# orybkin/video-gcp

Measured on AMD Instinct MI355X. Metric: predicted frames/sec, 64x64x3 seq_len=80 gcp_tree (posterior forward + all loss terms, model(inputs) and model.loss() of train.py:157-159, batch-stat BatchNorm), higher is better.
Workload: dtype f32 (encoder / decoder convs and the tree GEMMs from 512 rows: split-f16 MFMA with f32 accumulate, f32-equivalent; everything else exact f32 MFMA)

## Files before the change

### video-gcp_amd/csrc/conv3x3_split.hip

```cpp
#include "common.h"
#include "split_mfma.h"

#include <cstdlib>
#include <type_traits>

namespace {

struct SplitUpCfg {
    static constexpr int RW = 18, RH = 6, LW = 10, LH = 4, CC = 16, KS = 5;
    static constexpr int RAW_BYTES = LH * LW * CC * 4;
    static constexpr int PLANE_BYTES = RH * RW * 32;
    static constexpr int WAVE_BYTES = RAW_BYTES + 2 * PLANE_BYTES;
    static constexpr int NS = (LH * LW * 4 + 63) / 64;
    static constexpr int W_CHUNK_BYTES = KS * 2 * 1024;
    static int lds_bytes(int nchunk) { return nchunk * W_CHUNK_BYTES + 8 * WAVE_BYTES + 8 * 2 * 16 * 4; }
};

__global__ void __launch_bounds__(512, 2) conv3x3_up16_split_kernel(const gcpx_conv_args a, const int items_per_wave,
                                                                    const int nitems) {
    using Cfg = SplitUpCfg;
    constexpr int RW = Cfg::RW, RH = Cfg::RH, LW = Cfg::LW, LH = Cfg::LH, CC = Cfg::CC, NS = Cfg::NS, KS = Cfg::KS;
    extern __shared__ float4 smem4[];
    const int nchunk = a.Cin / CC;
    const char* wl = reinterpret_cast<const char*>(smem4);
// ... 163 lines not shown
            const int which = tid >> 4, c = tid & 15;
            float sum = 0.f;
#pragma unroll
            for (int w = 0; w < 8; ++w) sum += red[(w * 2 + which) * 16 + c];
            a.stats_partial[((size_t)blockIdx.x * 2 + which) * 16 + c] = sum;
        }
    }
}

template <int TILE> struct SplitTileShape;
template <> struct SplitTileShape<1> { static constexpr int TH = 16, TW = 16, TF = 1; };
template <> struct SplitTileShape<2> { static constexpr int TH = 8, TW = 8, TF = 4; };

template <int CT, int TILE>
struct SplitTileCfg {
    using TS = SplitTileShape<TILE>;
    static constexpr int TH = TS::TH, TW = TS::TW, TF = TS::TF, CC = 32, C4 = 8;
    static constexpr int RH = TH + 2, RW = TW + 2, LH = TH / 2 + 2, LW = TW / 2 + 2;
    static constexpr int PLANE_BYTES = TF * RH * RW * 64;
    static constexpr int RAW_BYTES = TF * LH * LW * CC * 4;
    static constexpr int LDS_BYTES = 2 * PLANE_BYTES + RAW_BYTES + 64;
    static constexpr int NSLOT = TF * LH * LW * C4;
    static constexpr int NS = (NSLOT + 255) / 256;
    static constexpr int PR = TH * TW * TF / 64;
};

template <int CT, int TILE>
__global__ void __launch_bounds__(256, 2) conv3x3_up32_split_kernel(const gcpx_conv_args a, const int ntx, const int nty, const int ntiles) {
    using Cfg = SplitTileCfg<CT, TILE>;
    constexpr int PR = Cfg::PR, TH = Cfg::TH, TW = Cfg::TW, TF = Cfg::TF, RH = Cfg::RH, RW = Cfg::RW;
    constexpr int LH = Cfg::LH, LW = Cfg::LW, CC = Cfg::CC, C4 = Cfg::C4, NS = Cfg::NS, NSLOT = Cfg::NSLOT;
    static_assert(PR == 4, "256 output pixels per workgroup");
    extern __shared__ float4 smem4[];
    char* hi = reinterpret_cast<char*>(smem4);
    float* raw = reinterpret_cast<float*>(hi + 2 * Cfg::PLANE_BYTES);
    float* wmax = reinterpret_cast<float*>(hi + 2 * Cfg::PLANE_BYTES + Cfg::RAW_BYTES);

    const int tid = threadIdx.x;
    const int lane = tid & 63, wave = tid >> 6;
    const int j = lane & 15, q = lane >> 4;
    const int nchunk = a.Cin / CC;
    const int Hout = a.Hout, Wout = a.Wout, F = a.F;
    const int ew = a.w_split_log2_dev ? __builtin_amdgcn_readfirstlane(*a.w_split_log2_dev) : a.w_split_log2;

    int pixoff[PR], pfl[PR], py[PR], px[PR];
#pragma unroll
    for (int pt = 0; pt < PR; ++pt) {
        const int p = (wave * PR + pt) * 16 + j;
        pfl[pt] = p / (TH * TW);
        const int rem = p % (TH * TW);
        py[pt] = rem / TW;
        px[pt] = rem % TW;
        pixoff[pt] = ((pfl[pt] * RH + py[pt]) * RW + px[pt]) * 64 + q * 16;
    }
    auto slot = [&](int k, int& c4, int& rx, int& ry, int& fl, int& lds) {
        const int idx = tid + 256 * k;
        c4 = idx % C4;
        int t = idx / C4;
        rx = t % LW; t /= LW;
        ry = t % LH;
        fl = (idx < NSLOT) ? t / LH : -1;
        lds = ((fl * LH + ry) * LW + rx) * CC + c4 * 4;
    };
    const char* wbase = reinterpret_cast<const char*>(a.wpk_split) + lane * 16;
    const int nstep = nchunk * 9;

    f32x4 st1[CT], st2[CT];
#pragma unroll
    for (int ct = 0; ct < CT; ++ct) { st1[ct] = f32x4{0, 0, 0, 0}; st2[ct] = f32x4{0, 0, 0, 0}; }

    float4 pre[NS];
    unsigned pre_ok = 0;
    auto tile_origin = [&](int tile, int& f0, int& y0, int& x0) {
        const int tx = tile % ntx;
        const int t2 = tile / ntx;
        f0 = (t2 / nty) * TF; y0 = (t2 % nty) * TH; x0 = tx * TW;
    };
    auto issue_loads = [&](int tile, int chunk) {
        int f0, y0, x0;
        tile_origin(tile, f0, y0, x0);
        pre_ok = 0;
        const int c0 = a.src[0].C;
#pragma unroll
        for (int k = 0; k < NS; ++k) {
            pre[k] = make_float4(0.f, 0.f, 0.f, 0.f);
            int s_c4, s_rx, s_ry, s_fl, s_lds;
            slot(k, s_c4, s_rx, s_ry, s_fl, s_lds);
            if (s_fl < 0) continue;
            const int f = f0 + s_fl;
            if (f < F) {
                const int sy = min(max(y0 / 2 - 1 + s_ry, 0), a.Hin - 1);
                const int sx = min(max(x0 / 2 - 1 + s_rx, 0), a.Win - 1);
                const int cg = chunk * CC + s_c4 * 4;
                const bool first = cg < c0;
                const gcpx_conv_src& sr = first ? a.src[0] : a.src[1];
                const int cl = first ? cg : cg - c0;
                pre[k] = *reinterpret_cast<const float4*>(sr.ptr + (((size_t)(f / sr.frame_div) * a.Hin + sy) * a.Win + sx) * sr.C + cl);
                pre_ok |= 1u << k;
            }
        }
    };

    int tile = blockIdx.x;
    if (tile < ntiles) issue_loads(tile, 0);
    for (; tile < ntiles; tile += gridDim.x) {
        int f0, y0, x0;
        tile_origin(tile, f0, y0, x0);
        f32x4 acc[CT][PR];
#pragma unroll
        for (int ct = 0; ct < CT; ++ct)
#pragma unroll
            for (int pt = 0; pt < PR; ++pt) acc[ct][pt] = f32x4{0, 0, 0, 0};
        int ex = 0;
        const bool top = (y0 == 0), bot = (y0 + TH == Hout), lft = (x0 == 0), rgt = (x0 + TW == Wout);

        h8 wr[3][CT][2];
        auto wload = [&](const int stn_, h8 (&w)[CT][2]) __attribute__((always_inline)) {
            const char* wp = wbase + (size_t)min(stn_, nstep - 1) * CT * 2048;
#pragma unroll
            for (int ct = 0; ct < CT; ++ct) {
                w[ct][0] = *reinterpret_cast<const h8*>(wp + ct * 2048);
                w[ct][1] = *reinterpret_cast<const h8*>(wp + ct * 2048 + 1024);
            }
        };
        if constexpr (CT <= 2) {
            wload(0, wr[0]);
            wload(1, wr[1]);
        }

        for (int chunk = 0; chunk < nchunk; ++chunk) {
            float amax = 0.f;
            {
                const int c0 = a.src[0].C;
#pragma unroll
                for (int k = 0; k < NS; ++k) {
                    int s_c4, s_rx, s_ry, s_fl, s_lds;
                    slot(k, s_c4, s_rx, s_ry, s_fl, s_lds);
                    if (s_fl < 0) continue;
                    float4 v = pre[k];
                    if (pre_ok & (1u << k)) {
                        const int cg = chunk * CC + s_c4 * 4;
                        const bool first = cg < c0;
                        const gcpx_conv_src& sr = first ? a.src[0] : a.src[1];
                        v = affine_act4(v, sr.scale, sr.shift, first ? cg : cg - c0, sr.act);
                    }
                    *reinterpret_cast<float4*>(raw + s_lds) = v;
                    amax = fmaxf(amax, fmaxf(fmaxf(fabsf(v.x), fabsf(v.y)), fmaxf(fabsf(v.z), fabsf(v.w))));
                }
            }
#pragma unroll
            for (int m = 1; m < 64; m <<= 1) amax = fmaxf(amax, __shfl_xor(amax, m));
            if (lane == 0) wmax[wave] = amax;
            __syncthreads();
            amax = fmaxf(fmaxf(wmax[0], wmax[1]), fmaxf(wmax[2], wmax[3]));
            int ec = 14 + 127 - (int)((__float_as_uint(amax) >> 23) & 0xff);
            ec = __builtin_amdgcn_readfirstlane(amax > 0.f ? max(-100, min(min(100, 126 - ew), ec)) : min(100, 126 - ew));
            if (chunk == 0) ex = ec;
            else if (ec < ex) {
                const float r = __uint_as_float((unsigned)(127 + ec - ex) << 23);
#pragma unroll
                for (int ct = 0; ct < CT; ++ct)
#pragma unroll
                    for (int pt = 0; pt < PR; ++pt) acc[ct][pt] *= r;
                ex = ec;
            }
            const float sx2 = __uint_as_float((unsigned)(127 + ex) << 23);
            {
                const int c4 = tid & (C4 - 1);
                const int p = tid >> 3;
                constexpr int RPP = 32 / (TW * TF);
                const int fl = (TF > 1) ? p / TW : 0;
                const int rx = p % TW;
                const int rsub = (RPP == 2) ? (p / TW) : 0;
                auto lerp_store = [&](int f2, int ry, int cx, bool zero) {
                    const float wx1 = (cx & 1) ? 0.75f : 0.25f, wx0 = 1.f - wx1;
                    const float wy1 = ((ry & 1) ? 0.75f : 0.25f), wy0 = 1.f - wy1;
                    const float* r = raw + ((f2 * LH + (ry >> 1)) * LW + (cx >> 1)) * CC + c4 * 4;
                    const float4 a00 = *reinterpret_cast<const float4*>(r);
                    const float4 a01 = *reinterpret_cast<const float4*>(r + CC);
                    const float4 a10 = *reinterpret_cast<const float4*>(r + LW * CC);
                    const float4 a11 = *reinterpret_cast<const float4*>(r + LW * CC + CC);
                    float4 v;
                    v.x = wy0 * (wx0 * a00.x + wx1 * a01.x) + wy1 * (wx0 * a10.x + wx1 * a11.x);
                    v.y = wy0 * (wx0 * a00.y + wx1 * a01.y) + wy1 * (wx0 * a10.y + wx1 * a11.y);
// ... 5 lines not shown
                    p1[0] = (_Float16)v.x; p1[1] = (_Float16)v.y; p1[2] = (_Float16)v.z; p1[3] = (_Float16)v.w;
                    p2[0] = (_Float16)(v.x - (float)p1[0]); p2[1] = (_Float16)(v.y - (float)p1[1]);
                    p2[2] = (_Float16)(v.z - (float)p1[2]); p2[3] = (_Float16)(v.w - (float)p1[3]);
                    char* dst = hi + ((f2 * RH + ry) * RW + cx) * 64 + c4 * 8;
                    *reinterpret_cast<h4*>(dst) = p1;
                    *reinterpret_cast<h4*>(dst + Cfg::PLANE_BYTES) = p2;
                };
#pragma unroll 2
                for (int k = 0; k < RH / RPP; ++k) {
                    const int ry = k * RPP + rsub;
                    lerp_store(fl, ry, rx + 1, (top && ry == 0) || (bot && ry == RH - 1));
                }
                for (int e = p; e < TF * RH * 2; e += 32) {
                    const int side = e & 1;
                    const int ry = (e >> 1) % RH, f2 = (e >> 1) / RH;
                    lerp_store(f2, ry, side ? RW - 1 : 0,
                               (top && ry == 0) || (bot && ry == RH - 1) || (lft && side == 0) || (rgt && side == 1));
                }
            }
            __syncthreads();
            if (chunk + 1 < nchunk) issue_loads(tile, chunk + 1);
            else if (tile + (int)gridDim.x < ntiles) issue_loads(tile + gridDim.x, 0);

            if constexpr (CT <= 2) {
                auto tap_mfmas = [&](const int tap, const h8 (&wc)[CT][2]) __attribute__((always_inline)) {
                    const int tapoff = ((tap / 3) * RW + (tap % 3)) * 64;
                    h8 b1[PR], b2[PR];
    #pragma unroll
                    for (int pt = 0; pt < PR; ++pt) {
                        b1[pt] = *reinterpret_cast<const h8*>(hi + pixoff[pt] + tapoff);
                        b2[pt] = *reinterpret_cast<const h8*>(hi + pixoff[pt] + tapoff + Cfg::PLANE_BYTES);
                    }
    #pragma unroll
                    for (int ct = 0; ct < CT; ++ct) {
    #pragma unroll
                        for (int pt = 0; pt < PR; ++pt) acc[ct][pt] = mfma32h(wc[ct][1], b1[pt], acc[ct][pt]);
    #pragma unroll
                        for (int pt = 0; pt < PR; ++pt) acc[ct][pt] = mfma32h(wc[ct][0], b2[pt], acc[ct][pt]);
    #pragma unroll
                        for (int pt = 0; pt < PR; ++pt) acc[ct][pt] = mfma32h(wc[ct][0], b1[pt], acc[ct][pt]);
                    }
                };
                __builtin_amdgcn_s_setprio(1);
    #pragma unroll 1
                for (int t3 = 0; t3 < 9; t3 += 3) {
                    wload(chunk * 9 + t3 + 2, wr[2]);
                    tap_mfmas(t3, wr[0]);
                    wload(chunk * 9 + t3 + 3, wr[0]);
                    tap_mfmas(t3 + 1, wr[1]);
                    wload(chunk * 9 + t3 + 4, wr[1]);
                    tap_mfmas(t3 + 2, wr[2]);
                }
            } else {
                h8 wn[CT][2];
                {
                    const char* wp = wbase + (size_t)(chunk * 9) * CT * 2048;
    #pragma unroll
                    for (int ct = 0; ct < CT; ++ct) {
                        wn[ct][0] = *reinterpret_cast<const h8*>(wp + ct * 2048);
                        wn[ct][1] = *reinterpret_cast<const h8*>(wp + ct * 2048 + 1024);
                    }
                }
                __builtin_amdgcn_s_setprio(1);
    #pragma unroll 1
                for (int tap = 0; tap < 9; ++tap) {
                    const int tapoff = ((tap / 3) * RW + (tap % 3)) * 64;
                    h8 wc[CT][2];
    #pragma unroll
                    for (int ct = 0; ct < CT; ++ct) { wc[ct][0] = wn[ct][0]; wc[ct][1] = wn[ct][1]; }
                    {
                        const int stn = min(chunk * 9 + tap + 1, nstep - 1);
                        const char* wp = wbase + (size_t)stn * CT * 2048;
    #pragma unroll
                        for (int ct = 0; ct < CT; ++ct) {
                            wn[ct][0] = *reinterpret_cast<const h8*>(wp + ct * 2048);
                            wn[ct][1] = *reinterpret_cast<const h8*>(wp + ct * 2048 + 1024);
                        }
                    }
                    h8 b1[PR], b2[PR];
    #pragma unroll
                    for (int pt = 0; pt < PR; ++pt) {
                        b1[pt] = *reinterpret_cast<const h8*>(hi + pixoff[pt] + tapoff);
                        b2[pt] = *reinterpret_cast<const h8*>(hi + pixoff[pt] + tapoff + Cfg::PLANE_BYTES);
                    }
    #pragma unroll
                    for (int ct = 0; ct < CT; ++ct) {
    #pragma unroll
                        for (int pt = 0; pt < PR; ++pt) acc[ct][pt] = mfma32h(wc[ct][1], b1[pt], acc[ct][pt]);
    #pragma unroll
                        for (int pt = 0; pt < PR; ++pt) acc[ct][pt] = mfma32h(wc[ct][0], b2[pt], acc[ct][pt]);
    #pragma unroll
                        for (int pt = 0; pt < PR; ++pt) acc[ct][pt] = mfma32h(wc[ct][0], b1[pt], acc[ct][pt]);
                    }
                }
            }
            __builtin_amdgcn_s_setprio(0);
        }

        const float inv = __uint_as_float((unsigned)(127 - ex - ew) << 23);
#pragma unroll
        for (int pt = 0; pt < PR; ++pt) {
            const int f = f0 + pfl[pt];
            if (f >= F) continue;
            float* op = a.out + (((size_t)f * Hout + (y0 + py[pt])) * Wout + (x0 + px[pt])) * a.out_pitch;
#pragma unroll
            for (int ct = 0; ct < CT; ++ct) {
                const float4 bv = *reinterpret_cast<const float4*>(a.bias + ct * 16 + q * 4);
                f32x4 v = acc[ct][pt];
                v[0] = fmaf(v[0], inv, bv.x); v[1] = fmaf(v[1], inv, bv.y); v[2] = fmaf(v[2], inv, bv.z); v[3] = fmaf(v[3], inv, bv.w);
                if (a.addend) {
                    const float4 ad = *reinterpret_cast<const float4*>(a.addend + (((size_t)(f / a.addend_frame_div) * Hout + (y0 + py[pt])) * Wout +
                                                                                   (x0 + px[pt])) * a.out_pitch + ct * 16 + q * 4);
                    v[0] += ad.x; v[1] += ad.y; v[2] += ad.z; v[3] += ad.w;
                }
                *reinterpret_cast<float4*>(op + ct * 16 + q * 4) = make_float4(v[0], v[1], v[2], v[3]);
                if (a.stats_partial) {
                    st1[ct] += v;
                    st2[ct] += v * v;
                }
            }
        }
    }

    if (a.stats_partial) {
        __syncthreads();
        float* red = reinterpret_cast<float*>(hi);
#pragma unroll
        for (int ct = 0; ct < CT; ++ct) {
#pragma unroll
            for (int r = 0; r < 4; ++r) {
                const float s1 = row16_sum(st1[ct][r]);
                const float s2 = row16_sum(st2[ct][r]);
                if (j == 0) {
                    red[(wave * 2 + 0) * CT * 16 + ct * 16 + q * 4 + r] = s1;
                    red[(wave * 2 + 1) * CT * 16 + ct * 16 + q * 4 + r] = s2;
                }
            }
        }
        __syncthreads();
        if (tid < 2 * CT * 16) {
            const int which = tid / (CT * 16), c = tid % (CT * 16);
            float sum = 0.f;
#pragma unroll
            for (int w = 0; w < 4; ++w) sum += red[(w * 2 + which) * CT * 16 + c];
            a.stats_partial[((size_t)blockIdx.x * 2 + which) * CT * 16 + c] = sum;
        }
    }
}

template <int CT, int TILE>
int launch_up32_split(const gcpx_conv_args* a, hipStream_t stream, int grid) {
    using Cfg = SplitTileCfg<CT, TILE>;
    const int ntx = a->Wout / Cfg::TW, nty = a->Hout / Cfg::TH;
    const int nfg = (a->F + Cfg::TF - 1) / Cfg::TF;
    auto kern = conv3x3_up32_split_kernel<CT, TILE>;
    static bool attr_set = false;
    if (!attr_set) {
        hipError_t e = hipFuncSetAttribute(reinterpret_cast<const void*>(kern), hipFuncAttributeMaxDynamicSharedMemorySize, Cfg::LDS_BYTES);
        if (e != hipSuccess) {
            gcpx_set_error("conv3x3 split up32: hipFuncSetAttribute(%d B LDS): %s", Cfg::LDS_BYTES, hipGetErrorString(e));
            return GCPX_ERR_HIP;
        }
        attr_set = true;
    }
    hipLaunchKernelGGL(kern, dim3(grid), dim3(256), Cfg::LDS_BYTES, stream, *a, ntx, nty, ntx * nty * nfg);
    GCPX_CHECK_LAUNCH();
    return GCPX_OK;
// ... 946 lines not shown
```

### video-gcp_amd/forward_plan.py

```python
import ctypes as C
import os
from contextlib import contextmanager

import torch

from . import packing as pk
from . import runtime as rt
from .hparams import GCPHParams
from .params import init_params, encoder_layers, encoder_skip_layers, decoder_layers
from .plan_ops import _Plan, _addr, N_LANES


class ForwardPlanMixin:

    def _plan_encoder(self, plan, tag, x_ptr, F, out_ptr, out_ob, out_orow, out_rpb):
        hp, P, lib = self._hp, self.pk, self.lib
        G = lib.gcpx_conv4x4s2_grid()
        S = hp.img_sz
        skip_idx = encoder_skip_layers(hp)
        skips = {}
        a0 = self._buf(f"{tag}.a0", (F, S // 2, S // 2, hp.ngf))
        enc_rec = dict(F=F, x_ptr=x_ptr, a0=a0, r={}, out=(out_ptr, out_ob, out_orow, out_rpb))
        plan.rec[f"enc:{tag}"] = enc_rec
        plan.add(f"enc.input:{tag}", lib.gcpx_conv4x4s2_image, x_ptr, P["enc.input.w"].data_ptr(),
# ... 47 lines not shown
        T, nz, dk = hp.max_seq_len, hp.nz_enc, hp.nz_attn_key
        li = l if hp.untied_layers else 0
        qin = self._buf(f"attn.qin{l}", (M, dk))
        self._mlp(plan, f"attn.query{l}", W["attn.query"], [el, er], M, n, out=qin.data_ptr(), ob=n * dk, orow=dk)
        dense = lambda t, w: self._rowsrc(t.data_ptr(), 0, w, w)
        qp = self._buf(f"attn.q{l}", (M, dk))
        self._gemm(plan, f"attn.q_proj{l}", [dense(qin, dk)], M, dk, M, W["attn.q_proj.w"], W["attn.q_proj.b"],
                   out=qp.data_ptr(), ob=0, orow=dk)
        o = self._buf(f"attn.o{l}", (M, nz))
        gamma = self._buf(f"attn.gamma{l}", (M, T))
        temp = self.sd[f"tree_module.tree_modules.{li}.inference.attention.attention_layers.0.temperature"]
        plan.add(f"attn{l}", lib.gcpx_attention, qp.data_ptr(), _addr(Kp, li * B * T * dk), _addr(Vp, li * B * T * nz), None,
                 tin["end_ind"].data_ptr(), temp.data_ptr(), o.data_ptr(), gamma.data_ptr(), M, n, T, dk, nz, hp.n_attention_heads)
        raw = self._buf(f"attn.raw{l}", (M, nz))
        self._gemm(plan, f"attn.out_proj{l}", [dense(o, nz)], M, nz, M, W["attn.out_proj.w"], W["attn.out_proj.b"],
                   out=raw.data_ptr(), ob=0, orow=nz)
        et = self._buf(f"attn.e_tilde{l}", (M, nz))
        self._gemm(plan, f"attn.out{l}", [dense(raw, nz)], M, nz, M, W["attn.out.w"], W["attn.out.b"], out=et.data_ptr(), ob=0, orow=nz)
        plan.rec.setdefault("gamma", {})[l] = gamma
        plan.rec.setdefault("e_tilde", {})[l] = et
        plan.rec.setdefault("attn", {})[l] = dict(qin=qin, qp=qp, o=o, raw=raw, gamma=gamma, et=et, M=M, n=n, li=li, temp=temp)
        return self._rowsrc(et.data_ptr(), n * nz, nz, nz)

    def _plan_decoder_features(self, plan, e_src, F, rpb, skips):
        hp, P, lib = self._hp, self.pk, self.lib
        ctop = self._c_top
        d0 = self._buf("dec.d0", (F, 4, 4, ctop))
        plan.rec["dec"] = dict(F=F, rpb=rpb, e_src=e_src, d0=d0, blocks=[], skips=skips)
        nrb = lib.gcpx_gemm_row_blocks(F, 16 * ctop)
        st = self._buf("dec.st0", (nrb, 2, 16 * ctop)) if self.training else None
        self._gemm(plan, "dec.input", [e_src], F, 16 * ctop, rpb, P["dec.input.w"], P["dec.input.b"], out=d0.data_ptr(),
                   ob=rpb * 16 * ctop, orow=16 * ctop, stats=st)
        sc, sh = self._bn(plan, "dec.bn0", "decoder.net.input.norm", ctop, st, nrb, 16 * ctop, F * 16)
        prev = (d0.data_ptr(), ctop, 1, sc, sh, rt.ACT_LRELU)
        res = 4
        for name, c_prev, c_skip, skip_idx, cout in decoder_layers(hp):
            srcs = [prev]
            if skip_idx >= 0:
                t, C_, ssc, ssh, sact = skips[skip_idx]
                assert C_ == c_skip and t.shape[1] == res
                srcs.append((t.data_ptr(), C_, rpb, ssc, ssh, sact))
            o = self._buf(f"dec.{name}", (F, 2 * res, 2 * res, cout))
            cpad = (cout + 15) // 16 * 16
            hoist = (skip_idx >= 0 and rpb > 1 and F % rpb == 0 and self.split_f16 and cout in (32, 64) and c_prev % 32 == 0 and
                     c_skip % 32 == 0 and f"dec.{name}" in self.pk_split and "fold" not in self.pk_split[f"dec.{name}"] and
                     os.environ.get("GCPX_NO_SKIP_HOIST") is None)
            hoist16 = (skip_idx >= 0 and rpb > 1 and F % rpb == 0 and self.split_f16 and cout == 16 and c_prev == 16 and c_skip == 16 and
                       f"dec.{name}.f16a" in self.pk_split and res % 4 == 0 and os.environ.get("GCPX_NO_SKIP_HOIST") is None)
            addend = None
            if hoist or hoist16:
                addend = self._buf(f"dec.{name}.skip", (F // rpb, 2 * res, 2 * res, cout))
                t, C_, ssc, ssh, sact = skips[skip_idx]
                zb = self._buf(f"dec.{name}.zero_bias", (cpad,), zero=True)
                a_s = self._conv_args([(t.data_ptr(), C_, 1, ssc, ssh, sact)], F // rpb, res, res, 2 * res, 2 * res, cout, cout,
                                      P[f"dec.{name}.w"], zb, addend, upsample=1)
                if hoist16:
                    self._set_split(a_s, f"dec.{name}.f16b")
                else:
                    self._set_split(a_s, f"dec.{name}")
                    a_s.wpk_split = a_s.wpk_split + (c_prev // 32) * 9 * (cpad // 16) * 2048
                plan.keep.append(a_s)
                plan.add(f"dec.{name}.skip", lib.gcpx_conv3x3, C.byref(a_s))
                srcs_main = [prev]
            else:
                srcs_main = srcs
            a = self._conv_args(srcs_main, F, res, res, 2 * res, 2 * res, cout, cout, P[f"dec.{name}.w"], P[f"dec.{name}.b"],
                                o, upsample=1, stats=(o if self.training else None))
            if hoist or hoist16:
                a.addend, a.addend_frame_div = addend.data_ptr(), rpb
            self._set_split(a, f"dec.{name}.f16a" if hoist16 else f"dec.{name}")
            Gl = lib.gcpx_conv3x3_grid(C.byref(a))
            assert Gl > 0, rt.lib().gcpx_last_error()
            st = self._buf(f"dec.st.{name}", (Gl, 2, cpad)) if self.training else None
            a.stats_partial = st.data_ptr() if st is not None else None
            plan.keep.append(a)
            plan.add(f"dec.{name}", lib.gcpx_conv3x3, C.byref(a))
            plan.rec["dec"]["blocks"].append(dict(name=name, srcs=srcs, out=o, res_in=res, cout=cout, c_prev=c_prev, c_skip=c_skip,
                                                  skip_idx=skip_idx))
            res *= 2
            sc, sh = self._bn(plan, f"dec.bn.{name}", f"decoder.net.{name}.norm", cout, st, Gl, cpad, F * res * res)
            prev = (o.data_ptr(), cout, 1, sc, sh, rt.ACT_LRELU)
        assert res == hp.img_sz
        return prev

    def _build_plan(self, key, tin):
        hp, P, lib = self._hp, self.pk, self.lib
        B, has_traj, has_z, sample_prior, phase, pred_len = key.B, key.has_traj, key.has_z, key.sample_prior, key.phase, key.pred_len
        train_aux = has_traj and phase == "train" and not sample_prior
        L, T, N = hp.hierarchy_levels, hp.max_seq_len, hp.n_nodes
        nz, nv, H, SD = hp.nz_enc, hp.nz_vae, hp.nz_mid_lstm, hp.lstm_state_dim
        PS = 2 ** L + 1
        plan = _Plan(lib)
        G = lib.gcpx_conv_grid()
# ... 55 lines not shown
                    else:
                        kenc = self._buf("inf_key_enc", (B * T, nz))
                        self._plan_seq_encoder(plan, "kseq", "inf_key_encoder.0", enc_traj, kenc, B)
                    keys = self._buf("inf_enc_key_seq", (B * T, dk))
                    dense = lambda t, w: self._rowsrc(t.data_ptr(), 0, w, w)
                    self._gemm(plan, "kseq.key", [dense(kenc, nz)], B * T, dk, B * T, P["kseq.key.w"], P["kseq.key.b"],
                               out=keys.data_ptr(), ob=0, orow=dk)
                    Kp = self._buf("attn.K", (n_mod, B * T, dk))
                    Vp = self._buf("attn.V", (n_mod, B * T, nz))
                    self._gemm(plan, "attn.k_proj", [dense(keys, dk)], B * T, dk, B * T, P["attn.k_proj.w"], P["attn.k_proj.b"],
                               out=Kp.data_ptr(), ob=0, orow=dk, batch=(n_mod, 0, P["attn.k_proj.w"][0].numel(), dk, B * T * dk))
                    self._gemm(plan, "attn.v_proj", [dense(inf_enc, nz)], B * T, nz, B * T, P["attn.v_proj.w"], P["attn.v_proj.b"],
                               out=Vp.data_ptr(), ob=0, orow=nz, batch=(n_mod, 0, P["attn.v_proj.w"][0].numel(), nz, B * T * nz))
                    plan.rec["attn_kv"] = dict(Kp=Kp, Vp=Vp, keys=keys, kenc=kenc, n_mod=n_mod)

        if traj_first:
            plan_traj_encoder()
        plan.lane = 1
        if "rng_all" in tin:
            plan.add("randn", lib.gcpx_randn, tin["rng_all"].data_ptr(), tin["rng_all"].numel(), self._buf("rng_state", (2,), torch.int64).data_ptr())
            if "aux_n" in tin and not pred_len:
                plan.wait(2, 1)
        skips = self._plan_encoder(plan, "I0", tin["I_0"].data_ptr(), B, _addr(E), PS * nz, 0, 1)
        plan.lane = 2
        if not pred_len:
            if "aux_n" in tin:
                plan_aux_indices()
            plan_bookkeeping()
        if hp.attach_cost_mdl and hp.run_cost_mdl and train_aux and self._has_aux_training:
            gt = self._buf("cost_target", (B,))
            rows = hp.input_nc * hp.img_sz
            plan.add("path_cost", lib.gcpx_path_cost, tin["traj_seq"].data_ptr(), tin["cost_start_idx"].data_ptr(),
                     tin["cost_end_idx"].data_ptr(), B, T, rows, hp.img_sz, self._buf("cost_partial", (B, rows)).data_ptr(), gt.data_ptr())
        self._plan_encoder(plan, "Ig", tin["I_g"].data_ptr(), B, _addr(E, 2 ** L * nz), PS * nz, 0, 1)
        outs = {}
        e0 = lambda: self._rowsrc(_addr(E), PS * nz, 0, nz)
        eg = lambda: self._rowsrc(_addr(E, 2 ** L * nz), PS * nz, 0, nz)
        if hp.regress_length and not pred_len:
            plan.wait(2, 1)
            logits = self._buf("seq_len_logits", (B, T))
            self._mlp(plan, "length_pred", P["length_pred"], [e0(), eg()], B, 1, out=logits.data_ptr(), ob=T, orow=0)
            outs["seq_len_logits"] = logits
        if not traj_first:
            plan_traj_encoder()
        plan.lane = 0
        plan.join([1, 2])
# ... 191 lines not shown
            la.seq_len = seq_len.data_ptr()
            if "actions_sampled" in outs and "actions" in tin:
                la.action_pred, la.action_seq, la.inv_t0 = outs["actions_sampled"].data_ptr(), tin["actions"].data_ptr(), tin["inv_t0"].data_ptr()
                la.n_actions, la.w_action = hp.n_actions, hp.action_rec_weight
            if "cost_pred" in outs:
                la.cost_pred, la.cost_target, la.w_cost = outs["cost_pred"].data_ptr(), outs["cost_target"].data_ptr(), 1.0
            loss_out = self._buf("losses", (16,), zero=True)
            la.out, la.B, la.T, la.N, la.state_dim = loss_out.data_ptr(), B, T, (N - 1 if adaptive else N), hp.state_dim
            la.w_rec, la.w_kl, la.w_len, la.w_exist, la.w_state = hp.dense_img_rec_weight, hp.kl_weight, hp.length_pred_weight, 1.0, 1.0
            if self._kl_w is not None:
                la.w_kl_dev = self._kl_w.data_ptr()
            la.total_div = float(T * hp.input_nc * hp.img_sz * hp.img_sz)
            plan.keep.append(la)
            return la, kl_b

        decode, with_loss = key.decode, key.with_loss
        loss_pre = None
        if with_loss and not adaptive:
            loss_pre = loss_args()
            plan.add("loss.pre", lib.gcpx_loss_pre, C.byref(loss_pre[0]), *kl_args(loss_pre[1]))
        if decode:
            F = B * N
            S = hp.img_sz
            prev = self._plan_decoder_features(plan, self._rowsrc(_addr(E, nz), PS * nz, nz, nz), F, N, skips)
            images = self._buf("images_df", (B, N, hp.input_nc, S, S))
            distr = matched_distr = None
            dlm = hp.decoder_distribution == "discrete_logistic_mixture"
            head_out, row_map = None, None
            fused_nll = None
            if dlm:
                mode = rt.HEAD_DLM_MEAN
                if self.materialize_distr or (adaptive and self.save_for_backward and with_loss):
                    mode, distr = rt.HEAD_DLM_BOTH, self._buf("distr_df", (B, N, S, S, self._head_pitch))
                    head_out = distr
                elif self._head_grad_fused(key):
                    mode, row_map = rt.HEAD_DLM_NLL_GRAD, node2row
                    head_out = self._buf("bw.dMD", (B * T, S, S, self._head_pitch))
                    fused_nll = self._buf("nll_partial", ((S // 4) * (S // 16), B * T), zero=True)
                    plan.rec["nll_bwd_fused"] = plan.rec["head_grad_fused"] = True
                elif with_loss and not adaptive and not self.save_for_backward and self._head_nll_fusable():
                    mode, row_map = rt.HEAD_DLM_NLL, node2row
                    fused_nll = self._buf("nll_partial", ((S // 4) * (S // 16), B * T), zero=True)
                elif with_loss and not adaptive:
                    mode, matched_distr = rt.HEAD_DLM_BOTH, self._buf("matched_distr", (B, T, S, S, self._head_pitch))
                    head_out, row_map = matched_distr, node2row
            else:
                mode = rt.HEAD_TANH_NCHW
# ... 122 lines not shown
```

### video-gcp_amd/sequential.py

```python
import ctypes as C
import os

import torch

from . import runtime as rt
from .model import GCPTreeModel, Outputs, _Plan, _addr
from .params import init_params_sequential


class GCPSequentialModel(GCPTreeModel):
    _has_aux_training = True
    _has_pred_length = False
    _rng_in_plan = False
    _has_training = True

    def _check_hp(self, hp):
        assert hp.lstm_init in ("zero", "mlp")
        assert hp.n_actions <= 16 or not hp.action_conditioned_pred, "the action rows are padded to one 16-column k-group"

    @property
    def _nets(self):
        return ("gen_lstm",) if self._hp.deterministic else ("prior_lstm", "inf_lstm", "gen_lstm")

    def _default_params(self, hp, seed):
# ... 131 lines not shown
        hp, P, lib = self._hp, self.pk, self.lib
        B, has_traj, has_z, sample_prior, phase, with_loss = key.B, key.has_traj, key.has_z, key.sample_prior, key.phase, key.with_loss
        T, nz, nv, H, nl = hp.max_seq_len, hp.nz_enc, hp.nz_vae, hp.nz_mid_lstm, hp.n_lstm_layers
        S = hp.img_sz
        plan = _Plan(lib)
        X = self._buf("seq.X", (B, T, nz))
        EG = self._buf("seq.EG", (B, nz))
        PZ = self._buf("seq.PZ", (B, T - 1, 2 * nv))
        QZ = self._buf("seq.QZ", (B, T - 1, 2 * nv), zero=True)
        Z = self._buf("seq.Z", (B, T - 1, nv))
        idx = self._buf("seq.idx", (B, T), torch.int32)
        seq_len = self._buf("seq.len", (B,), torch.int32)
        plan.add("seq_index", lib.gcpx_seq_index, tin["end_ind"].data_ptr(), B, T, idx.data_ptr(), seq_len.data_ptr())
        train_aux = has_traj and phase == "train" and not sample_prior
        if "aux_n" in tin:
            AUXK = ("inv_t0", "inv_t1", "cost_start_idx", "cost_end_idx")
            plan.add("aux_sample_indices", lib.gcpx_aux_sample_indices_gauss, tin["end_ind"].data_ptr(), tin["aux_n"].data_ptr(), B,
                     hp.inv_mdl_temp_dist, *[tin[k].data_ptr() for k in AUXK])

        enc_traj = None
        plan.fork([1, 2])
        plan.lane = 1
        skips = self._plan_encoder(plan, "I0", tin["I_0"].data_ptr(), B, _addr(X), T * nz, 0, 1)
        plan.lane = 2
        if hp.attach_cost_mdl and hp.run_cost_mdl and train_aux and "cost_start_idx" in tin:
            rows = hp.input_nc * hp.img_sz
            plan.add("path_cost", lib.gcpx_path_cost, tin["traj_seq"].data_ptr(), tin["cost_start_idx"].data_ptr(),
                     tin["cost_end_idx"].data_ptr(), B, T, rows, hp.img_sz, self._buf("cost_partial", (B, rows)).data_ptr(),
                     self._buf("cost_target", (B,)).data_ptr())
        self._plan_encoder(plan, "Ig", tin["I_g"].data_ptr(), B, _addr(EG), nz, 0, 1)
        plan.lane = 0
        if has_traj:
            enc_traj = self._buf("enc_traj", (B * T, nz))
            self._plan_encoder(plan, "traj", tin["traj_seq"].data_ptr(), B * T, enc_traj.data_ptr(), T * nz, nz, T)
        plan.join([1, 2])
        outs = {}
        e0 = lambda: self._rowsrc(_addr(X), T * nz, 0, nz)
        eg = lambda: self._rowsrc(_addr(EG), nz, 0, nz)
        if hp.regress_length:
            logits = self._buf("seq_len_logits", (B, T))
            self._mlp(plan, "length_pred", P["length_pred"], [e0(), eg()], B, 1, out=logits.data_ptr(), ob=T, orow=0)
            outs["seq_len_logits"] = logits

        EA = None
        if hp.action_conditioned_pred:
            na = hp.n_actions
# ... 174 lines not shown
            first = enc_traj if has_traj else mes
            s0 = self._rowsrc(first.data_ptr(), T * nz, nz, nz)
            s1 = self._rowsrc(_addr(mes, nz), T * nz, nz, nz)
            self._mlp(plan, "inv_mdl", P["inv_mdl"], [s0, s1], B * (T - 1), T - 1, out=act.data_ptr(),
                      ob=(T - 1) * hp.n_actions, orow=hp.n_actions)
            outs["actions_padded"] = act
        if aux_ok and ((hp.attach_inv_mdl and not hp.train_inv_mdl_full_seq) or (hp.attach_cost_mdl and hp.run_cost_mdl)):
            aux_rows = self._buf("aux_rows", (4, B), torch.int32)
            plan.add("aux_index_rows", lib.gcpx_aux_index_rows, tin["inv_t0"].data_ptr(), tin["inv_t1"].data_ptr(),
                     tin["cost_start_idx"].data_ptr(), tin["cost_end_idx"].data_ptr(), B, T, T, aux_rows.data_ptr())
            gather = lambda t, i: self._rowsrc(t.data_ptr(), 0, nz, nz, rowidx=aux_rows[i])
            if hp.attach_inv_mdl and not hp.train_inv_mdl_full_seq:
                act = self._buf("actions_sampled", (B, hp.n_actions))
                self._mlp(plan, "inv_mdl", P["inv_mdl"], [gather(enc_traj, 0), gather(mes, 1)], B, B, out=act.data_ptr(), ob=0,
                          orow=hp.n_actions)
                outs["actions_sampled"] = act
            if hp.attach_cost_mdl and hp.run_cost_mdl:
                cost = self._buf("cost_pred", (B, 1))
                self._mlp(plan, "cost_mdl", P["cost_mdl"], [gather(mes, 2), gather(mes, 3)], B, B, out=cost.data_ptr(), ob=0, orow=1)
                outs["cost_pred"], outs["cost_target"] = cost, self._buf("cost_target", (B,))
        plan.lane = 0

        F = B * (T - 1)
        prev = self._plan_decoder_features(plan, self._rowsrc(_addr(X, nz), T * nz, nz, nz), F, T - 1, skips)
        dec_images = self._buf("seq.dec_images", (B, T - 1, hp.input_nc, S, S))
        dlm = hp.decoder_distribution == "discrete_logistic_mixture"
        head_out = row_map = matched = fused_nll = None
        if dlm:
            mode = rt.HEAD_DLM_MEAN
            if with_loss or self.materialize_distr:
                row_map = self._buf("seq.row_map", (F,), torch.int32)
                row_map.copy_((torch.arange(B)[:, None] * T + torch.arange(1, T)[None]).reshape(-1).to(torch.int32))
                if with_loss and self._head_nll_fusable():
                    fused_nll = self._buf("nll_partial", ((S // 4) * (S // 16), B * T), zero=True)
                    mode = rt.HEAD_DLM_NLL
                    if self.save_for_backward:
                        mode, head_out = rt.HEAD_DLM_NLL_GRAD, self._buf("bw.dMD", (B * T, S, S, self._head_pitch))
                        r2f = self._buf("seq.row2frame", (B * T,), torch.int32)
                        inv = torch.arange(B * T, dtype=torch.int64).view(B, T) // T * (T - 1) + torch.arange(T)[None] - 1
                        inv[:, 0] = -1
                        r2f.copy_(inv.reshape(-1).to(torch.int32))
                        plan.add("zero_unmapped", lib.gcpx_zero_unmapped_rows, head_out.data_ptr(), S * S * self._head_pitch,
                                 r2f.data_ptr(), B * T)
                        plan.rec["nll_bwd_fused"] = plan.rec["head_grad_fused"] = True
                else:
                    mode, matched = rt.HEAD_DLM_BOTH, self._buf("matched_distr", (B, T, S, S, self._head_pitch))
                    head_out = matched
# ... 123 lines not shown
```

Before: 503,700.

## Split up32 conv output channels across wavefronts and hoist decoder skip convs earlier

The 32-channel upsample conv kernel now splits output-channel tiles across wavefronts when CT>=4, so each wave holds fewer accumulators and runs the same three-tap weight-prefetch pipeline that was previously limited to CT<=2. Pixel offsets are computed from a single base plus compile-time group offsets, which cuts per-pixel register state. Separately, the skip-half convolutions of the decoder are scheduled right after the I0 encoder on its lane, so they can overlap with other work instead of sitting inline in the decoder chain. The costs are more duplicated LDS B-fragment reads per wave and a more complicated indexing scheme.

```diff
diff --git a/video-gcp_amd/csrc/conv3x3_split.hip b/video-gcp_amd/csrc/conv3x3_split.hip
--- a/video-gcp_amd/csrc/conv3x3_split.hip
+++ b/video-gcp_amd/csrc/conv3x3_split.hip
@@ -209,7 +209,15 @@
     static constexpr int LDS_BYTES = 2 * PLANE_BYTES + RAW_BYTES + 64;
     static constexpr int NSLOT = TF * LH * LW * C4;
     static constexpr int NS = (NSLOT + 255) / 256;
-    static constexpr int PR = TH * TW * TF / 64;
+    static constexpr int CW = CT >= 4 ? 2 : 1;
+    static constexpr int CH = CT / CW;
+    static constexpr int PW = 4 / CW;
+    static constexpr int PR = TH * TW * TF / 16 / PW;
+    static constexpr int GPF = TH * TW / 16;
+    static constexpr int RPG = 16 / TW;
+    static constexpr int gfl(int g) { return g / GPF; }
+    static constexpr int gy(int g) { return (g % GPF) * RPG; }
+    static constexpr int goff(int g) { return (gfl(g) * RH + gy(g)) * RW * 64; }
 };
 
 template <int CT, int TILE>
@@ -217,31 +225,27 @@
     using Cfg = SplitTileCfg<CT, TILE>;
     constexpr int PR = Cfg::PR, TH = Cfg::TH, TW = Cfg::TW, TF = Cfg::TF, RH = Cfg::RH, RW = Cfg::RW;
     constexpr int LH = Cfg::LH, LW = Cfg::LW, CC = Cfg::CC, C4 = Cfg::C4, NS = Cfg::NS, NSLOT = Cfg::NSLOT;
-    static_assert(PR == 4, "256 output pixels per workgroup");
+    constexpr int CH = Cfg::CH, CW = Cfg::CW, PW = Cfg::PW;
+    static_assert(PR * PW == 16 && CH * CW == CT && PR % 4 == 0 && (PR % Cfg::GPF == 0 || Cfg::GPF % PR == 0), "CW x PW wavefronts over 256 output pixels");
     extern __shared__ float4 smem4[];
     char* hi = reinterpret_cast<char*>(smem4);
     float* raw = reinterpret_cast<float*>(hi + 2 * Cfg::PLANE_BYTES);
     float* wmax = reinterpret_cast<float*>(hi + 2 * Cfg::PLANE_BYTES + Cfg::RAW_BYTES);
 
     const int tid = threadIdx.x;
-    const int lane = tid & 63, wave = tid >> 6;
+    const int lane = tid & 63, wave = __builtin_amdgcn_readfirstlane(tid >> 6);
+    const int cw = wave % CW, pw = wave / CW;
     const int j = lane & 15, q = lane >> 4;
     const int nchunk = a.Cin / CC;
     const int Hout = a.Hout, Wout = a.Wout, F = a.F;
     const int ew = a.w_split_log2_dev ? __builtin_amdgcn_readfirstlane(*a.w_split_log2_dev) : a.w_split_log2;
 
-    int pixoff[PR], pfl[PR], py[PR], px[PR];
-#pragma unroll
-    for (int pt = 0; pt < PR; ++pt) {
-        const int p = (wave * PR + pt) * 16 + j;
-        pfl[pt] = p / (TH * TW);
-        const int rem = p % (TH * TW);
-        py[pt] = rem / TW;
-        px[pt] = rem % TW;
-        pixoff[pt] = ((pfl[pt] * RH + py[pt]) * RW + px[pt]) * 64 + q * 16;
-    }
+    const int fl0 = pw * PR / Cfg::GPF, py0 = pw * PR % Cfg::GPF * Cfg::RPG + j / TW, px0 = j % TW;
+    const int pix0 = ((fl0 * RH + py0) * RW + px0) * 64 + q * 16;
     auto slot = [&](int k, int& c4, int& rx, int& ry, int& fl, int& lds) {
-        const int idx = tid + 256 * k;
+        int t_ = tid;
+        if constexpr (CT > 2) asm volatile("" : "+v"(t_));
+        const int idx = t_ + 256 * k;
         c4 = idx % C4;
         int t = idx / C4;
         rx = t % LW; t /= LW;
@@ -249,12 +253,13 @@
         fl = (idx < NSLOT) ? t / LH : -1;
         lds = ((fl * LH + ry) * LW + rx) * CC + c4 * 4;
     };
-    const char* wbase = reinterpret_cast<const char*>(a.wpk_split) + lane * 16;
+    const char* wbase = reinterpret_cast<const char*>(a.wpk_split) + cw * CH * 2048 + lane * 16;
     const int nstep = nchunk * 9;
-
-    f32x4 st1[CT], st2[CT];
-#pragma unroll
-    for (int ct = 0; ct < CT; ++ct) { st1[ct] = f32x4{0, 0, 0, 0}; st2[ct] = f32x4{0, 0, 0, 0}; }
+    const int cbase = cw * CH * 16 + q * 4;
+
+    f32x4 st1[CH], st2[CH];
+#pragma unroll
+    for (int ct = 0; ct < CH; ++ct) { st1[ct] = f32x4{0, 0, 0, 0}; st2[ct] = f32x4{0, 0, 0, 0}; }
 
     float4 pre[NS];
     unsigned pre_ok = 0;
@@ -293,27 +298,25 @@
     for (; tile < ntiles; tile += gridDim.x) {
         int f0, y0, x0;
         tile_origin(tile, f0, y0, x0);
-        f32x4 acc[CT][PR];
-#pragma unroll
-        for (int ct = 0; ct < CT; ++ct)
+        f32x4 acc[CH][PR];
+#pragma unroll
+        for (int ct = 0; ct < CH; ++ct)
 #pragma unroll
             for (int pt = 0; pt < PR; ++pt) acc[ct][pt] = f32x4{0, 0, 0, 0};
         int ex = 0;
         const bool top = (y0 == 0), bot = (y0 + TH == Hout), lft = (x0 == 0), rgt = (x0 + TW == Wout);
 
-        h8 wr[3][CT][2];
-        auto wload = [&](const int stn_, h8 (&w)[CT][2]) __attribute__((always_inline)) {
+        h8 wr[3][CH][2];
+        auto wload = [&](const int stn_, h8 (&w)[CH][2]) __attribute__((always_inline)) {
             const char* wp = wbase + (size_t)min(stn_, nstep - 1) * CT * 2048;
 #pragma unroll
-            for (int ct = 0; ct < CT; ++ct) {
+            for (int ct = 0; ct < CH; ++ct) {
                 w[ct][0] = *reinterpret_cast<const h8*>(wp + ct * 2048);
                 w[ct][1] = *reinterpret_cast<const h8*>(wp + ct * 2048 + 1024);
             }
         };
-        if constexpr (CT <= 2) {
-            wload(0, wr[0]);
-            wload(1, wr[1]);
-        }
+        wload(0, wr[0]);
+        wload(1, wr[1]);
 
         for (int chunk = 0; chunk < nchunk; ++chunk) {
             float amax = 0.f;
@@ -346,7 +349,7 @@
             else if (ec < ex) {
                 const float r = __uint_as_float((unsigned)(127 + ec - ex) << 23);
 #pragma unroll
-                for (int ct = 0; ct < CT; ++ct)
+                for (int ct = 0; ct < CH; ++ct)
 #pragma unroll
                     for (int pt = 0; pt < PR; ++pt) acc[ct][pt] *= r;
                 ex = ec;
@@ -398,77 +401,36 @@
             if (chunk + 1 < nchunk) issue_loads(tile, chunk + 1);
             else if (tile + (int)gridDim.x < ntiles) issue_loads(tile + gridDim.x, 0);
 
-            if constexpr (CT <= 2) {
-                auto tap_mfmas = [&](const int tap, const h8 (&wc)[CT][2]) __attribute__((always_inline)) {
-                    const int tapoff = ((tap / 3) * RW + (tap % 3)) * 64;
-                    h8 b1[PR], b2[PR];
-    #pragma unroll
-                    for (int pt = 0; pt < PR; ++pt) {
-                        b1[pt] = *reinterpret_cast<const h8*>(hi + pixoff[pt] + tapoff);
-                        b2[pt] = *reinterpret_cast<const h8*>(hi + pixoff[pt] + tapoff + Cfg::PLANE_BYTES);
+            auto tap_mfmas = [&](const char* bp, const h8 (&wc)[CH][2]) __attribute__((always_inline)) {
+                static_for<0, PR / 4>([&](auto hc) __attribute__((always_inline)) {
+                    constexpr int g0 = decltype(hc)::value * 4;
+                    h8 b1[4], b2[4];
+                    static_for<0, 4>([&](auto ic) __attribute__((always_inline)) {
+                        constexpr int i = decltype(ic)::value;
+                        b1[i] = *reinterpret_cast<const h8*>(bp + Cfg::goff(g0 + i));
+                        b2[i] = *reinterpret_cast<const h8*>(bp + Cfg::goff(g0 + i) + Cfg::PLANE_BYTES);
+                    });
+#pragma unroll
+                    for (int ct = 0; ct < CH; ++ct) {
+#pragma unroll
+                        for (int i = 0; i < 4; ++i) acc[ct][g0 + i] = mfma32h(wc[ct][1], b1[i], acc[ct][g0 + i]);
+#pragma unroll
+                        for (int i = 0; i < 4; ++i) acc[ct][g0 + i] = mfma32h(wc[ct][0], b2[i], acc[ct][g0 + i]);
+#pragma unroll
+                        for (int i = 0; i < 4; ++i) acc[ct][g0 + i] = mfma32h(wc[ct][0], b1[i], acc[ct][g0 + i]);
                     }
-    #pragma unroll
-                    for (int ct = 0; ct < CT; ++ct) {
-    #pragma unroll
-                        for (int pt = 0; pt < PR; ++pt) acc[ct][pt] = mfma32h(wc[ct][1], b1[pt], acc[ct][pt]);
-    #pragma unroll
-                        for (int pt = 0; pt < PR; ++pt) acc[ct][pt] = mfma32h(wc[ct][0], b2[pt], acc[ct][pt]);
-    #pragma unroll
-                        for (int pt = 0; pt < PR; ++pt) acc[ct][pt] = mfma32h(wc[ct][0], b1[pt], acc[ct][pt]);
-                    }
-                };
-                __builtin_amdgcn_s_setprio(1);
-    #pragma unroll 1
-                for (int t3 = 0; t3 < 9; t3 += 3) {
-                    wload(chunk * 9 + t3 + 2, wr[2]);
-                    tap_mfmas(t3, wr[0]);
-                    wload(chunk * 9 + t3 + 3, wr[0]);
-                    tap_mfmas(t3 + 1, wr[1]);
-                    wload(chunk * 9 + t3 + 4, wr[1]);
-                    tap_mfmas(t3 + 2, wr[2]);
-                }
-            } else {
-                h8 wn[CT][2];
-                {
-                    const char* wp = wbase + (size_t)(chunk * 9) * CT * 2048;
-    #pragma unroll
-                    for (int ct = 0; ct < CT; ++ct) {
-                        wn[ct][0] = *reinterpret_cast<const h8*>(wp + ct * 2048);
-                        wn[ct][1] = *reinterpret_cast<const h8*>(wp + ct * 2048 + 1024);
-                    }
-                }
-                __builtin_amdgcn_s_setprio(1);
-    #pragma unroll 1
-                for (int tap = 0; tap < 9; ++tap) {
-                    const int tapoff = ((tap / 3) * RW + (tap % 3)) * 64;
-                    h8 wc[CT][2];
-    #pragma unroll
-                    for (int ct = 0; ct < CT; ++ct) { wc[ct][0] = wn[ct][0]; wc[ct][1] = wn[ct][1]; }
-                    {
-                        const int stn = min(chunk * 9 + tap + 1, nstep - 1);
-                        const char* wp = wbase + (size_t)stn * CT * 2048;
-    #pragma unroll
-                        for (int ct = 0; ct < CT; ++ct) {
-                            wn[ct][0] = *reinterpret_cast<const h8*>(wp + ct * 2048);
-                            wn[ct][1] = *reinterpret_cast<const h8*>(wp + ct * 2048 + 1024);
-                        }
-                    }
-                    h8 b1[PR], b2[PR];
-    #pragma unroll
-                    for (int pt = 0; pt < PR; ++pt) {
-                        b1[pt] = *reinterpret_cast<const h8*>(hi + pixoff[pt] + tapoff);
-                        b2[pt] = *reinterpret_cast<const h8*>(hi + pixoff[pt] + tapoff + Cfg::PLANE_BYTES);
-                    }
-    #pragma unroll
-                    for (int ct = 0; ct < CT; ++ct) {
-    #pragma unroll
-                        for (int pt = 0; pt < PR; ++pt) acc[ct][pt] = mfma32h(wc[ct][1], b1[pt], acc[ct][pt]);
-    #pragma unroll
-                        for (int pt = 0; pt < PR; ++pt) acc[ct][pt] = mfma32h(wc[ct][0], b2[pt], acc[ct][pt]);
-    #pragma unroll
-                        for (int pt = 0; pt < PR; ++pt) acc[ct][pt] = mfma32h(wc[ct][0], b1[pt], acc[ct][pt]);
-                    }
-                }
+                });
+            };
+            __builtin_amdgcn_s_setprio(1);
+#pragma unroll 1
+            for (int t3 = 0; t3 < 9; t3 += 3) {
+                const char* bp = hi + pix0 + (t3 / 3) * RW * 64;
+                wload(chunk * 9 + t3 + 2, wr[2]);
+                tap_mfmas(bp, wr[0]);
+                wload(chunk * 9 + t3 + 3, wr[0]);
+                tap_mfmas(bp + 64, wr[1]);
+                wload(chunk * 9 + t3 + 4, wr[1]);
+                tap_mfmas(bp + 128, wr[2]);
             }
             __builtin_amdgcn_s_setprio(0);
         }
@@ -476,20 +438,21 @@
         const float inv = __uint_as_float((unsigned)(127 - ex - ew) << 23);
 #pragma unroll
         for (int pt = 0; pt < PR; ++pt) {
-            const int f = f0 + pfl[pt];
+            const int f = f0 + fl0 + Cfg::gfl(pt);
             if (f >= F) continue;
-            float* op = a.out + (((size_t)f * Hout + (y0 + py[pt])) * Wout + (x0 + px[pt])) * a.out_pitch;
-#pragma unroll
-            for (int ct = 0; ct < CT; ++ct) {
-                const float4 bv = *reinterpret_cast<const float4*>(a.bias + ct * 16 + q * 4);
+            const int oy = y0 + py0 + Cfg::gy(pt), ox = x0 + px0;
+            float* op = a.out + (((size_t)f * Hout + oy) * Wout + ox) * a.out_pitch + cbase;
+#pragma unroll
+            for (int ct = 0; ct < CH; ++ct) {
+                const float4 bv = *reinterpret_cast<const float4*>(a.bias + cbase + ct * 16);
                 f32x4 v = acc[ct][pt];
                 v[0] = fmaf(v[0], inv, bv.x); v[1] = fmaf(v[1], inv, bv.y); v[2] = fmaf(v[2], inv, bv.z); v[3] = fmaf(v[3], inv, bv.w);
                 if (a.addend) {
-                    const float4 ad = *reinterpret_cast<const float4*>(a.addend + (((size_t)(f / a.addend_frame_div) * Hout + (y0 + py[pt])) * Wout +
-                                                                                   (x0 + px[pt])) * a.out_pitch + ct * 16 + q * 4);
+                    const float4 ad = *reinterpret_cast<const float4*>(a.addend + (((size_t)(f / a.addend_frame_div) * Hout + oy) * Wout + ox) *
+                                                                                      a.out_pitch + cbase + ct * 16);
                     v[0] += ad.x; v[1] += ad.y; v[2] += ad.z; v[3] += ad.w;
                 }
-                *reinterpret_cast<float4*>(op + ct * 16 + q * 4) = make_float4(v[0], v[1], v[2], v[3]);
+                *reinterpret_cast<float4*>(op + ct * 16) = make_float4(v[0], v[1], v[2], v[3]);
                 if (a.stats_partial) {
                     st1[ct] += v;
                     st2[ct] += v * v;
@@ -502,14 +465,14 @@
         __syncthreads();
         float* red = reinterpret_cast<float*>(hi);
 #pragma unroll
-        for (int ct = 0; ct < CT; ++ct) {
+        for (int ct = 0; ct < CH; ++ct) {
 #pragma unroll
             for (int r = 0; r < 4; ++r) {
                 const float s1 = row16_sum(st1[ct][r]);
                 const float s2 = row16_sum(st2[ct][r]);
                 if (j == 0) {
-                    red[(wave * 2 + 0) * CT * 16 + ct * 16 + q * 4 + r] = s1;
-                    red[(wave * 2 + 1) * CT * 16 + ct * 16 + q * 4 + r] = s2;
+                    red[(pw * 2 + 0) * CT * 16 + cbase + ct * 16 + r] = s1;
+                    red[(pw * 2 + 1) * CT * 16 + cbase + ct * 16 + r] = s2;
                 }
             }
         }
@@ -518,7 +481,7 @@
             const int which = tid / (CT * 16), c = tid % (CT * 16);
             float sum = 0.f;
 #pragma unroll
-            for (int w = 0; w < 4; ++w) sum += red[(w * 2 + which) * CT * 16 + c];
+            for (int w = 0; w < PW; ++w) sum += red[(w * 2 + which) * CT * 16 + c];
             a.stats_partial[((size_t)blockIdx.x * 2 + which) * CT * 16 + c] = sum;
         }
     }
diff --git a/video-gcp_amd/forward_plan.py b/video-gcp_amd/forward_plan.py
--- a/video-gcp_amd/forward_plan.py
+++ b/video-gcp_amd/forward_plan.py
@@ -93,7 +93,43 @@
         plan.rec.setdefault("attn", {})[l] = dict(qin=qin, qp=qp, o=o, raw=raw, gamma=gamma, et=et, M=M, n=n, li=li, temp=temp)
         return self._rowsrc(et.data_ptr(), n * nz, nz, nz)
 
-    def _plan_decoder_features(self, plan, e_src, F, rpb, skips):
+    def _skip_hoist_kind(self, name, res, c_prev, c_skip, skip_idx, cout, F, rpb):
+        if skip_idx < 0 or rpb <= 1 or F % rpb or not self.split_f16 or os.environ.get("GCPX_NO_SKIP_HOIST") is not None:
+            return None
+        if (cout in (32, 64) and c_prev % 32 == 0 and c_skip % 32 == 0 and f"dec.{name}" in self.pk_split and
+                "fold" not in self.pk_split[f"dec.{name}"]):
+            return 32
+        if cout == 16 and c_prev == 16 and c_skip == 16 and f"dec.{name}.f16a" in self.pk_split and res % 4 == 0:
+            return 16
+        return None
+
+    def _plan_skip_half(self, plan, name, kind, res, c_prev, cout, skip, F, rpb):
+        P, lib = self.pk, self.lib
+        cpad = (cout + 15) // 16 * 16
+        addend = self._buf(f"dec.{name}.skip", (F // rpb, 2 * res, 2 * res, cout))
+        t, C_, ssc, ssh, sact = skip
+        zb = self._buf(f"dec.{name}.zero_bias", (cpad,), zero=True)
+        a_s = self._conv_args([(t.data_ptr(), C_, 1, ssc, ssh, sact)], F // rpb, res, res, 2 * res, 2 * res, cout, cout,
+                              P[f"dec.{name}.w"], zb, addend, upsample=1)
+        if kind == 16:
+            self._set_split(a_s, f"dec.{name}.f16b")
+        else:
+            self._set_split(a_s, f"dec.{name}")
+            a_s.wpk_split = a_s.wpk_split + (c_prev // 32) * 9 * (cpad // 16) * 2048
+        plan.keep.append(a_s)
+        plan.add(f"dec.{name}.skip", lib.gcpx_conv3x3, C.byref(a_s))
+        return addend
+
+    def _plan_decoder_skips(self, plan, F, rpb, skips):
+        addends, res = {}, 4
+        for name, c_prev, c_skip, skip_idx, cout in decoder_layers(self._hp):
+            kind = self._skip_hoist_kind(name, res, c_prev, c_skip, skip_idx, cout, F, rpb)
+            if kind:
+                addends[name] = self._plan_skip_half(plan, name, kind, res, c_prev, cout, skips[skip_idx], F, rpb)
+            res *= 2
+        return addends
+
+    def _plan_decoder_features(self, plan, e_src, F, rpb, skips, addends=None):
         hp, P, lib = self._hp, self.pk, self.lib
         ctop = self._c_top
         d0 = self._buf("dec.d0", (F, 4, 4, ctop))
@@ -113,33 +149,21 @@
                 srcs.append((t.data_ptr(), C_, rpb, ssc, ssh, sact))
             o = self._buf(f"dec.{name}", (F, 2 * res, 2 * res, cout))
             cpad = (cout + 15) // 16 * 16
-            hoist = (skip_idx >= 0 and rpb > 1 and F % rpb == 0 and self.split_f16 and cout in (32, 64) and c_prev % 32 == 0 and
-                     c_skip % 32 == 0 and f"dec.{name}" in self.pk_split and "fold" not in self.pk_split[f"dec.{name}"] and
-                     os.environ.get("GCPX_NO_SKIP_HOIST") is None)
-            hoist16 = (skip_idx >= 0 and rpb > 1 and F % rpb == 0 and self.split_f16 and cout == 16 and c_prev == 16 and c_skip == 16 and
-                       f"dec.{name}.f16a" in self.pk_split and res % 4 == 0 and os.environ.get("GCPX_NO_SKIP_HOIST") is None)
+            kind = self._skip_hoist_kind(name, res, c_prev, c_skip, skip_idx, cout, F, rpb)
             addend = None
-            if hoist or hoist16:
-                addend = self._buf(f"dec.{name}.skip", (F // rpb, 2 * res, 2 * res, cout))
-                t, C_, ssc, ssh, sact = skips[skip_idx]
-                zb = self._buf(f"dec.{name}.zero_bias", (cpad,), zero=True)
-                a_s = self._conv_args([(t.data_ptr(), C_, 1, ssc, ssh, sact)], F // rpb, res, res, 2 * res, 2 * res, cout, cout,
-                                      P[f"dec.{name}.w"], zb, addend, upsample=1)
-                if hoist16:
-                    self._set_split(a_s, f"dec.{name}.f16b")
+            if kind:
+                if addends is not None:
+                    addend = addends[name]
                 else:
-                    self._set_split(a_s, f"dec.{name}")
-                    a_s.wpk_split = a_s.wpk_split + (c_prev // 32) * 9 * (cpad // 16) * 2048
-                plan.keep.append(a_s)
-                plan.add(f"dec.{name}.skip", lib.gcpx_conv3x3, C.byref(a_s))
+                    addend = self._plan_skip_half(plan, name, kind, res, c_prev, cout, skips[skip_idx], F, rpb)
                 srcs_main = [prev]
             else:
                 srcs_main = srcs
             a = self._conv_args(srcs_main, F, res, res, 2 * res, 2 * res, cout, cout, P[f"dec.{name}.w"], P[f"dec.{name}.b"],
                                 o, upsample=1, stats=(o if self.training else None))
-            if hoist or hoist16:
+            if kind:
                 a.addend, a.addend_frame_div = addend.data_ptr(), rpb
-            self._set_split(a, f"dec.{name}.f16a" if hoist16 else f"dec.{name}")
+            self._set_split(a, f"dec.{name}.f16a" if kind == 16 else f"dec.{name}")
             Gl = lib.gcpx_conv3x3_grid(C.byref(a))
             assert Gl > 0, rt.lib().gcpx_last_error()
             st = self._buf(f"dec.st.{name}", (Gl, 2, cpad)) if self.training else None
@@ -241,6 +265,7 @@
             if "aux_n" in tin and not pred_len:
                 plan.wait(2, 1)
         skips = self._plan_encoder(plan, "I0", tin["I_0"].data_ptr(), B, _addr(E), PS * nz, 0, 1)
+        dec_addends = self._plan_decoder_skips(plan, B * N, N, skips) if key.decode else None
         plan.lane = 2
         if not pred_len:
             if "aux_n" in tin:
@@ -478,7 +503,7 @@
         if decode:
             F = B * N
             S = hp.img_sz
-            prev = self._plan_decoder_features(plan, self._rowsrc(_addr(E, nz), PS * nz, nz, nz), F, N, skips)
+            prev = self._plan_decoder_features(plan, self._rowsrc(_addr(E, nz), PS * nz, nz, nz), F, N, skips, addends=dec_addends)
             images = self._buf("images_df", (B, N, hp.input_nc, S, S))
             distr = matched_distr = None
             dlm = hp.decoder_distribution == "discrete_logistic_mixture"
diff --git a/video-gcp_amd/sequential.py b/video-gcp_amd/sequential.py
--- a/video-gcp_amd/sequential.py
+++ b/video-gcp_amd/sequential.py
@@ -177,6 +177,7 @@
         plan.fork([1, 2])
         plan.lane = 1
         skips = self._plan_encoder(plan, "I0", tin["I_0"].data_ptr(), B, _addr(X), T * nz, 0, 1)
+        dec_addends = self._plan_decoder_skips(plan, B * (T - 1), T - 1, skips)
         plan.lane = 2
         if hp.attach_cost_mdl and hp.run_cost_mdl and train_aux and "cost_start_idx" in tin:
             rows = hp.input_nc * hp.img_sz
@@ -397,7 +398,7 @@
         plan.lane = 0
 
         F = B * (T - 1)
-        prev = self._plan_decoder_features(plan, self._rowsrc(_addr(X, nz), T * nz, nz, nz), F, T - 1, skips)
+        prev = self._plan_decoder_features(plan, self._rowsrc(_addr(X, nz), T * nz, nz, nz), F, T - 1, skips, addends=dec_addends)
         dec_images = self._buf("seq.dec_images", (B, T - 1, hp.input_nc, S, S))
         dlm = hp.decoder_distribution == "discrete_logistic_mixture"
         head_out = row_map = matched = fused_nll = None
```

New measurement: 511,800, median of 6. +1.6%, better.
